# LemonATsu/UNet-PhaseGen

Measured on AMD Instinct MI355X. Metric: spectrogram-frames/sec (train fwd+bwd), higher is better.
Workload: dtype f32; 1 GPU; train.py full step (fwd + cos/sin/mag loss + bwd + Adam), UNetModel(1024, 2048), per-GPU batch 64 x 1024 bins x 256 frames (BASELINE configs[2]); global_batch=64, frames=256, channels=1024, parallelism=dp1, grad_allreduce_payload=fp32, adam=fused into the wgrad epilogues

## Files before the change

### include/phasegen.h

```cpp
#ifndef PHASEGEN_H
#define PHASEGEN_H
#include <stdint.h>

#ifdef __cplusplus
extern "C" {
#endif

#define PG_VERSION 400

enum { PG_OK = 0, PG_ERR_NULL = -1, PG_ERR_SHAPE = -2, PG_ERR_ALIGN = -3, PG_ERR_UNSUPPORTED = -4,
       PG_ERR_WORKSPACE = -5 };

enum { PG_ACT_NONE = 0, PG_ACT_LEAKY02 = 1 , PG_ACT_RELU = 2  };

struct pg_adam_args;
typedef struct pg_conv_args {
    int32_t B, Cin, Cout, Lin, Lout, k, stride, pad;
    const float* x;  int64_t x_bs;
    int32_t x_act;
    int32_t precision;
    const float* w;
    float* y;        int64_t y_bs;
    const float* dy; int64_t dy_bs;
    float* dx;       int64_t dx_bs;
    const float* dx_add; int64_t dx_add_bs;
    const float* dx_ref; int64_t dx_ref_bs;
    int32_t dx_mask;
    int32_t schedule;
    float* dw;
    int32_t y_act; int32_t y2_act;
    float* y2;       int64_t y2_bs;
    void* workspace; int64_t workspace_bytes;
    const struct pg_adam_args* adam;
} pg_conv_args;
int64_t pg_workspace_bytes_conv(void);
enum { PG_PREC_FP32 = 0, PG_PREC_BF16 = 1, PG_PREC_BF16X3 = 2 };
enum { PG_SCHED_AUTO = 0, PG_SCHED_TILE_PER_WG = 1, PG_SCHED_FORCE_STREAMK = 2, PG_SCHED_NO_RAW = 4, PG_SCHED_NO_TALL = 8,
       PG_SCHED_CONTENDED = 16, PG_SCHED_NO_PS = 128, PG_SCHED_NO_RAW3 = 0x2000, PG_SCHED_ALL_RAW3 = 0x4000, PG_SCHED_NO_COLSPLIT = 0x20000, PG_SCHED_COLSPLIT = 0x40000 };
#define PG_SCHED_OVERSUB(f) (((f) & 15) << 8)

int pg_conv1d_fwd(const pg_conv_args* a, void* stream);
int pg_conv1d_dgrad(const pg_conv_args* a, void* stream);
int pg_conv1d_wgrad(const pg_conv_args* a, void* stream);
int pg_convt1d_fwd(const pg_conv_args* a, void* stream);
int pg_convt1d_dgrad(const pg_conv_args* a, void* stream);
int pg_convt1d_wgrad(const pg_conv_args* a, void* stream);
enum { PG_OP_CONV1D_FWD = 0, PG_OP_CONV1D_DGRAD = 1, PG_OP_CONV1D_WGRAD = 2,
       PG_OP_CONVT1D_FWD = 3, PG_OP_CONVT1D_DGRAD = 4, PG_OP_CONVT1D_WGRAD = 5 };
int pg_conv_describe(const pg_conv_args* a, int32_t op, char* buf, int32_t buflen);

// ... 104 lines not shown
```

### unet-phasegen_amd/csrc/conv_common.h

```cpp
#pragma once
#include <hip/hip_runtime.h>
#include <stdint.h>
#include "phasegen.h"
#include "pg_common.h"

namespace pgconv {

struct IgemmParams {
    const float* x; long x_bs;
    const float* w;
    const float* pt; long pt_bs;
    float* y; long y_bs;
    const float* add; long add_bs;
    const float* ref; long ref_bs;
    unsigned x_bytes, w_bytes, pt_bytes;
    int B, Q, M, Lx, Ly, k, s, p;
    int act_x, act_p, mask_mode;
    int U, u_off;
    int LP; float inv_LP;
    int a_vec;
    int tilesM, tilesN;
    int g_ps;
    int tn_stride;
    float* y2; long y2_bs; float y_slope, y2_slope;
    float* ws;
    int nslab;
    int whole;
    int sr;
    int n_lo;
    int x_pitch;
    unsigned short* yh; long yh_bs; int yh_pitch; float yh_slope;
    unsigned short* yh2; long yh2_bs; int yh2_pitch; float yh2_slope;
    float* ad_p; float* ad_m; float* ad_v; PgAdamScalars ad;
};

}
using pgconv::IgemmParams;

namespace {


constexpr int WMB = 4;
constexpr int BM = 64 * WMB, BN = 128, BK = 16, NT = 256;
constexpr int TILE_A = BM * BK, TILE_B = BN * BK;
constexpr int STAGE = TILE_A + TILE_B;
constexpr int AE = BM / 16;

typedef float f32x16 __attribute__((ext_vector_type(16)));
// ... 387 lines not shown
#define PG_STAMP_FLUSH
#define PG_STAMP_DECL
#endif

__device__ __forceinline__ void divmod24(int n, int d, float inv, int& q, int& r) {
    q = (int)((float)n * inv);
    r = n - q * d;
    if (r < 0) { r += d; --q; }
    if (r >= d) { r -= d; ++q; }
}

constexpr int RBM = 128, RBN = 256;
constexpr int RS2 = 768, RS1 = 384;
constexpr int raw_gap(int tj) { return tj >= 8 ? 16 : tj; }
constexpr int RTILE_A = RBM * BK;

enum Kind { KIND_F, KIND_T, KIND_G };

}

namespace pgconv {
hipError_t launch_im2col(int kind, const IgemmParams& p, int grid, hipStream_t st, int prec);
hipError_t launch_raw_ft(int kind, const IgemmParams& p, int grid, hipStream_t st, int prec);
hipError_t launch_raw_ft_tall(int kind, const IgemmParams& p, int grid, hipStream_t st, int prec);
hipError_t launch_raw_g(const IgemmParams& p, int grid, hipStream_t st, int prec);
hipError_t launch_h3(int kind, const IgemmParams& p, int grid, hipStream_t st);
hipError_t launch_h3_fixup(int kind, const IgemmParams& p, int grid, unsigned split_tiles, bool wide, hipStream_t st);
bool raw3_covers(int kind, const IgemmParams& p);
hipError_t launch_raw3(int kind, const IgemmParams& p, int grid, hipStream_t st);
hipError_t launch_raw3_fixup(int kind, const IgemmParams& p, int grid, unsigned blocks, hipStream_t st);
// ... 3 lines not shown
```

### unet-phasegen_amd/csrc/conv_igemm.hip

```cpp
#include <hip/hip_runtime.h>
#include <cstring>
#include <cmath>
#include "conv_common.h"

namespace {

template <int KIND, int MB, int NB, int WN = 2, bool WIDE = false>
__global__ __launch_bounds__(NT) void conv_fixup_kernel(const IgemmParams p, int G) {
    __shared__ float red[WIDE ? 3 * 16 * 64 : 1];
    const int unit = WIDE ? blockIdx.x >> 2 : blockIdx.x, q = WIDE ? threadIdx.x >> 6 : 0;
    const int tid = WIDE ? (blockIdx.x & 3) * 64 + (threadIdx.x & 63) : threadIdx.x;
    const int lane = tid & 63, wv = tid >> 6;
    const int wm = WN == 2 ? wv >> 1 : (WN == 4 ? 0 : wv), wn = WN == 2 ? wv & 1 : (WN == 4 ? wv : 0);
    static_assert(MB * NB * 16 == ACC_REGS, "8 blocks per wave tile: the host launches 8 workgroups per tile");
    const int tile = p.whole + unit / (MB * NB), blk = unit % (MB * NB), bi = blk / NB, bj = blk - bi * NB;
    const Split sp = make_split(p.tilesM * p.tilesN, p.nslab, G, p.whole);
    const int first = tile * p.nslab, last = first + p.nslab - 1;
    const int g0 = split_owner(sp, first), g1 = split_owner(sp, last);
    if (g0 == g1 && split_lo(sp, g0) <= first && split_lo(sp, g0 + 1) > last) return;
    if (KIND != 2 && p.n_lo + (tile % p.tilesN) * p.tn_stride + (WN == 2 ? wn * (NB - 1) * 32 : (WN == 4 ? wn * (NB * 32) : 0)) + bj * 32 >= p.B * (KIND == 0 ? p.Ly : p.U)) return;
    AccT<1, 1> acc;
#pragma unroll
    for (int r = 0; r < 16; ++r) acc.c[0][0][r] = 0.f;
#pragma unroll 2
// ... 31 lines not shown

struct Knobs {
    int prec;
    int force_mode;
    int no_raw;
    int no_tall;
    int oversub;
    int contended;
    int no_ps;
    int no_raw3;
    int all_raw3;
    int sr;
    int force_colsplit;
    int no_colsplit;
    char* desc; int desc_len;
};
int decode_knobs(const pg_conv_args* a, Knobs& k) {
    if (a->precision < 0 || a->precision > 2) return pg_fail(PG_ERR_UNSUPPORTED, "conv: precision must be PG_PREC_FP32, PG_PREC_BF16 or PG_PREC_BF16X3");
    const int sc = a->schedule;
    if (sc < 0 || (sc & ~0x7ffff) || ((sc >> 17) & 3) == 3 || (sc & 3) == 3 || ((sc >> 8) & 15) > 8) return pg_fail(PG_ERR_SHAPE, "conv: bad schedule bits");
    k.prec = a->precision;
    k.force_mode = sc & 3; k.no_raw = (sc >> 2) & 1; k.no_tall = (sc >> 3) & 1;
    k.oversub = (sc >> 8) & 15; if (!k.oversub) k.oversub = 4;
    k.contended = (sc >> 4) & 1;
    if ((sc >> 5) & 3) return pg_fail(PG_ERR_UNSUPPORTED, "conv: schedule bits 5-6 (tile families removed in 0.4)");
    k.no_ps = (sc >> 7) & 1;
    k.no_raw3 = (sc >> 13) & 1;
    k.all_raw3 = (sc >> 14) & 1;
    k.sr = ((sc >> 15) & 3) ? 1 << (((sc >> 15) & 3) - 1) : 0;
    k.no_colsplit = (sc >> 17) & 1;
    k.force_colsplit = (sc >> 18) & 1;
    if (k.no_raw3 && k.all_raw3) return pg_fail(PG_ERR_SHAPE, "conv: schedule bits 13 and 14 exclude each other");
    k.desc = nullptr; k.desc_len = 0;
    return PG_OK;
}

int cu_count() { return pg_cu_count(); }
bool fixup_wide(int grid, long split_tiles) { return split_tiles > 0 && grid >= 8 * split_tiles; }

int pick_grid(long tiles, int nslab, IgemmParams& p, long ws_bytes, int mode, int oversub, int contended, int wg_per_cu = WG_PER_CU,
              long ws_per_wg = WS_PER_WG) {
    const long total = tiles * (long)nslab;
    const long slots = (long)cu_count() * wg_per_cu;
    p.whole = 0;
    if (mode == 0 && !contended && tiles % slots == 0) {
        if (tiles <= slots * oversub) return (int)tiles;
        for (long mult = oversub; mult >= 1; --mult)
            if (tiles % (slots * mult) == 0) return (int)(slots * mult);
// ... 25 lines not shown
    const bool k5 = p.k == 5 && p.s == 2;
    if (kind == KIND_F) {
        if (!((p.k == 32 && p.s == 2) || (p.k == 8 && p.s == 1) || (p.k == 8 && p.s == 2) || (p.k == 4 && p.s == 2) || (k5 && p.Q % 2 == 0))) return false;
        kwp = virtual_k(p.k, p.s); sc = p.s; lcol = p.Ly;
    } else if (kind == KIND_T) {
        if (!((p.k == 32 && p.s == 2) || (p.k == 8 && p.s == 1) || (p.k == 8 && p.s == 2) || (p.k == 4 && p.s == 2) || k5)) return false;
        kwp = virtual_k(p.k, p.s) / p.s; sc = 1; lcol = p.U;
    } else {
        return p.LP >= 16 && ((p.k == 32 && p.s == 2) || (p.k == 8 && p.s == 1) || (p.k == 8 && p.s == 2) || (p.k == 4 && p.s == 2) || k5);
    }
    const int tj = kwp < 16 ? kwp : 16;
    const int nseg_max = (lcol - 1 + tn - 1) / lcol + 1;
    return sc * (tn - 1) + tj + raw_gap(tj) * (nseg_max - 1) + (kind == KIND_T ? tj : 0) <= (sc == 1 ? RS1 : RS2);
}

int launch(Kind kind, IgemmParams& p, const Knobs& kn, long rows, long cols, long Ktot, long ws_bytes, hipStream_t st, bool may_split = true) {
    const long Ktot_in = Ktot;
    bool raw = raw_supported(kind, p, kn);
    const long cols_wide = (cols + RBN - 1) / RBN * RBN, cols_tall = (cols + RBN / 2 - 1) / (RBN / 2) * (RBN / 2);
    const bool tall = kind != KIND_G && kn.no_raw == 0 && kn.no_tall == 0 && (cols_tall * 100 <= cols_wide * 97 || !raw) &&
                      raw_supported(kind, p, kn, RBN / 2);
    if (tall) raw = true;
    const bool r3_over_tall = tall && raw_supported(kind, p, kn) && (kn.all_raw3 || cols_wide * 100 <= cols_tall * 108);
    const bool r3_ok = raw && raw_supported(kind, p, kn) && kind != KIND_G && kn.prec == 0 && !kn.no_raw3 && pgconv::raw3_covers(kind, p) &&
                       (rows + 255) / 256 * 256 * 100 <= (rows + RBM - 1) / RBM * RBM * 103;
    const bool r3 = r3_ok && (!tall || r3_over_tall);
    const int bm = (tall || r3) ? 2 * RBM : (raw ? RBM : BM);
    int bn = (tall && !r3) ? RBN / 2 : (raw ? RBN : BN);
    const bool k5 = raw && p.k == 5 && p.s == 2;
    if (k5 && kind == KIND_G) bn = (RBN / 5) * 5;
    p.g_ps = 0;
    if (raw && kind == KIND_G && p.k != 32) {
// ... 4 lines not shown
    if (may_split && r3_ok && kn.force_mode != 1 && !kn.no_colsplit && !kn.no_tall) {
        const long full = cols / RBN * RBN, rem = cols - full;
        if (full > 0 && rem > 0 && rem <= RBN / 2 && raw_supported(kind, p, kn, RBN / 2)) {
            const double rows_p = (double)((rows + 255) / 256 * 256), rem32 = (double)((rem + 31) / 32 * 32), Kd = (double)Ktot;
            const double t_col = 2.0 * rows_p * 256.0 * Kd / 140e6;
            const double t_tail = fmax(4.0 * (double)rows * Kd / 3e6, 2.0 * rows_p * rem32 * Kd / 100e6) + 25.0;
            IgemmParams pa = p;
            const long tiles_a = (rows + 255) / 256 * (full / RBN), nslab_a = (Ktot + BK - 1) / BK;
            const long grid_a = pick_grid(tiles_a, (int)nslab_a, pa, ws_bytes, kn.force_mode, kn.oversub, kn.contended, 1, 2 * WS_PER_WG);
            const bool aligned = pa.whole == 0 && (grid_a % tiles_a == 0 || tiles_a % grid_a == 0);
            if ((t_col > 1.3 * t_tail && aligned) || kn.force_colsplit) {
                Knobs kb = kn;
                kb.no_raw3 = 1; kb.all_raw3 = 0;
                char tail[160] = "";
                if (kn.desc) { kb.desc = tail; kb.desc_len = (int)sizeof tail; }
                int rc = launch(kind, p, kn, rows, full, Ktot_in, ws_bytes, st, false);
                if (rc != PG_OK) return rc;
                IgemmParams pb = p;
                pb.n_lo = (int)full;
                rc = launch(kind, pb, kb, rows, rem, Ktot_in, ws_bytes, st, false);
                if (rc == PG_OK && kn.desc) {
                    char* bar = strchr(tail, '|');
                    if (bar) { *bar = ','; bar = strchr(bar, '|'); if (bar) *bar = 0; }
                    const size_t n = strlen(kn.desc);
                    if (n + 7 < (size_t)kn.desc_len) snprintf(kn.desc + n, (size_t)kn.desc_len - n, "|tail=%s", tail);
                }
                return rc;
            }
        }
    }
    if (p.n_lo && !(tall && !r3)) return pg_fail(PG_ERR_UNSUPPORTED, "conv: internal -- a column tail off the tall tile");
    p.tn_stride = bn;
    p.sr = r3 ? (kn.sr ? kn.sr : (p.k == 8 ? 2 : 1)) : 0;
    p.tilesM = (int)((rows + bm - 1) / bm);
    p.tilesN = (int)((cols + bn - 1) / bn);
    p.nslab = (int)((Ktot + BK - 1) / BK);
    const long tiles = (long)p.tilesM * p.tilesN;
    if (tiles <= 0 || tiles > 0x0fffffffL || p.nslab <= 0 || cols + bn >= 0x7fffffffL) return pg_fail(PG_ERR_SHAPE, "conv: empty or oversize grid");
    const int grid = r3 ? pick_grid(tiles, p.nslab, p, ws_bytes, kn.force_mode, kn.oversub, kn.contended, 1, 2 * WS_PER_WG)
                        : pick_grid(tiles, p.nslab, p, ws_bytes, kn.force_mode, kn.oversub, kn.contended);
    const bool split = grid != tiles && !(tiles % grid == 0);
    if (kn.desc) {
        char name[96];
        if (raw && kind == KIND_G) snprintf(name, sizeof name, "conv_g_%s_kernel<%d, %d, %d>", p.g_ps ? "ps" : "raw", p.k, p.s, kn.prec);
        else if (r3) snprintf(name, sizeof name, "conv_raw3_kernel<%d, %d, %s, %s>", p.k, p.s, kind == KIND_T ? "true" : "false", p.act_x == PG_ACT_NONE ? "false" : "true");
        else if (raw) snprintf(name, sizeof name, "conv_raw_kernel<%d, %d, %s, %d, %d>", p.k, p.s, kind == KIND_T ? "true" : "false", kn.prec, tall ? 1 : 2);
        else snprintf(name, sizeof name, "conv_%c_kernel<0, 0, %d>", kind == KIND_F ? 'f' : (kind == KIND_T ? 't' : 'g'), kn.prec);
        snprintf(kn.desc, (size_t)kn.desc_len, "%s|grid=%d|tiles=%ld|slabs=%d|split=%d|whole=%d|fixup=%s", name, grid, tiles, p.nslab, (int)split, p.whole,
                 !split ? "none" : (!r3 && fixup_wide(grid, tiles - p.whole) ? "wide" : "plain"));
        return PG_OK;
    }
    hipError_t e;
    if (r3) e = pgconv::launch_raw3(kind, p, grid, st);
    else if (raw && kind == KIND_G) e = pgconv::launch_raw_g(p, grid, st, kn.prec);
    else if (tall) e = pgconv::launch_raw_ft_tall(kind, p, grid, st, kn.prec);
    else if (raw) e = pgconv::launch_raw_ft(kind, p, grid, st, kn.prec);
    else e = pgconv::launch_im2col(kind, p, grid, st, kn.prec);
    if (e == hipSuccess && split && r3) e = pgconv::launch_raw3_fixup(kind, p, grid, (unsigned)((tiles - p.whole) * 16), st);
    else if (e == hipSuccess && split) {
        const bool wide = fixup_wide(grid, tiles - p.whole);
        const dim3 fg((unsigned)((tiles - p.whole) * (wide ? 32 : 8)));
#define PG_FIXUP(...) { if (wide) hipLaunchKernelGGL((conv_fixup_kernel<__VA_ARGS__, true>), fg, dim3(NT), 0, st, p, grid); \
                        else hipLaunchKernelGGL((conv_fixup_kernel<__VA_ARGS__, false>), fg, dim3(NT), 0, st, p, grid); }
        if (tall) {
            if (kind == KIND_F) PG_FIXUP(0, 2, 4, 1)
// ... 118 lines not shown
}

static int set_fused_adam(IgemmParams& p, const pg_conv_args* a) {
    const pg_adam_args* ad = a->adam;
    if (!ad) return PG_OK;
    if (!ad->p || !ad->m || !ad->v) return pg_fail(PG_ERR_NULL, "wgrad: fused adam needs p, m and v");
    if (ad->step < 1) return pg_fail(PG_ERR_SHAPE, "wgrad: fused adam: step is 1-based");
    if (ad->n != (int64_t)a->Cin * a->Cout * a->k) return pg_fail(PG_ERR_SHAPE, "wgrad: fused adam: n must equal Cin * Cout * k (p / m / v shaped like dw)");
    if (((uintptr_t)ad->p | (uintptr_t)ad->m | (uintptr_t)ad->v) & 3) return pg_fail(PG_ERR_ALIGN, "wgrad: fused adam: misaligned pointer");
    if ((const float*)ad->p == a->dw || ad->m == a->dw || ad->v == a->dw) return pg_fail(PG_ERR_SHAPE, "wgrad: fused adam: p / m / v alias dw");
    p.ad_p = ad->p; p.ad_m = ad->m; p.ad_v = ad->v;
    p.ad = pg_adam_scalars(ad);
    return PG_OK;
}

static int run_conv1d_wgrad(const pg_conv_args* a, void* stream, char* desc, int desc_len) {
    if (int e = check_geom(a, false)) return e;
    Knobs kn; if (int e = decode_knobs(a, kn)) return e;
    kn.desc = desc; kn.desc_len = desc_len;
    if (!a->dy || !a->x || !a->dw) return pg_fail(PG_ERR_NULL, "conv1d_wgrad: dy, x, dw required");
    IgemmParams p = {};
    p.pt = a->dy; p.pt_bs = a->dy_bs; p.LP = a->Lout; p.act_p = PG_ACT_NONE;
    p.x = a->x; p.x_bs = a->x_bs; p.act_x = a->x_act; p.y = a->dw;
    p.B = a->B; p.Q = a->Cin; p.M = a->Cout; p.Lx = a->Lin; p.k = a->k; p.s = a->stride; p.p = a->pad;
    if (int e = set_extents(p, p.Q, p.Lx, p.M, p.LP)) return e;
    if (int e = set_fused_adam(p, a)) return e;
    p.ws = (float*)a->workspace;
    return launch(KIND_G, p, kn, p.M, (long)p.Q * p.k, (long)p.B * p.LP, a->workspace_bytes, (hipStream_t)stream);
}

static int run_convt1d_wgrad(const pg_conv_args* a, void* stream, char* desc, int desc_len) {
    if (int e = check_geom(a, true)) return e;
    Knobs kn; if (int e = decode_knobs(a, kn)) return e;
    kn.desc = desc; kn.desc_len = desc_len;
    if (!a->dy || !a->x || !a->dw) return pg_fail(PG_ERR_NULL, "convt1d_wgrad: dy, x, dw required");
    IgemmParams p = {};
    p.pt = a->x; p.pt_bs = a->x_bs; p.LP = a->Lin; p.act_p = a->x_act;
    p.x = a->dy; p.x_bs = a->dy_bs; p.act_x = PG_ACT_NONE; p.y = a->dw;
    p.B = a->B; p.Q = a->Cout; p.M = a->Cin; p.Lx = a->Lout; p.k = a->k; p.s = a->stride; p.p = a->pad;
    if (int e = set_extents(p, p.Q, p.Lx, p.M, p.LP)) return e;
    if (int e = set_fused_adam(p, a)) return e;
    p.ws = (float*)a->workspace;
    return launch(KIND_G, p, kn, p.M, (long)p.Q * p.k, (long)p.B * p.LP, a->workspace_bytes, (hipStream_t)stream);
}

extern "C" int pg_conv1d_fwd(const pg_conv_args* a, void* stream) { return run_conv1d_fwd(a, stream, nullptr, 0); }
extern "C" int pg_conv1d_dgrad(const pg_conv_args* a, void* stream) { return run_conv1d_dgrad(a, stream, nullptr, 0); }
extern "C" int pg_conv1d_wgrad(const pg_conv_args* a, void* stream) { return run_conv1d_wgrad(a, stream, nullptr, 0); }
extern "C" int pg_convt1d_fwd(const pg_conv_args* a, void* stream) { return run_convt1d_fwd(a, stream, nullptr, 0); }
extern "C" int pg_convt1d_dgrad(const pg_conv_args* a, void* stream) { return run_convt1d_dgrad(a, stream, nullptr, 0); }
// ... 48 lines not shown
        p.u_off = p.p / p.s;
        p.U = (p.Ly - 1 + p.p) / p.s - p.u_off + 1;
        if (p.U <= 0) return pg_fail(PG_ERR_SHAPE, "conv_fwd_h: empty output");
    }
    if (!pgconv::h_supported(kind, p)) return pg_fail(PG_ERR_UNSUPPORTED, "conv_fwd_h: geometry not covered by the bf16-resident kernels (use the fp32-tensor entry points)");
    if (query) return PG_OK;
    const long rows = tr ? (long)p.M * p.s : p.M, cols = (long)p.B * (tr ? p.U : p.Ly), Ktot = (long)p.Q * kwp;
    const int tm = 2 * RBM, tn = RBN;
    p.tilesM = (int)((rows + tm - 1) / tm);
    p.tilesN = (int)((cols + tn - 1) / tn);
    p.tn_stride = tn;
    p.nslab = (int)(Ktot / 32);
    p.ws = (float*)a->workspace;
    const long tiles = (long)p.tilesM * p.tilesN;
    if (tiles <= 0 || tiles > 0x0fffffffL || p.nslab <= 0) return pg_fail(PG_ERR_SHAPE, "conv_fwd_h: empty or oversize grid");
    const int grid = pick_grid(tiles, p.nslab, p, a->workspace_bytes, kn.force_mode, kn.oversub, kn.contended, 1, 2 * WS_PER_WG);
    const bool split = grid != tiles && !(tiles % grid == 0);
    if (desc) {
        snprintf(desc, (size_t)desc_len, "conv_h3_kernel<%d, %d, %s>|grid=%d|tiles=%ld|slabs=%d|split=%d|whole=%d|fixup=%s",
                 (tr && p.k == 5) ? 8 : p.k, p.s, tr ? "true" : "false", grid, tiles, p.nslab, (int)split, p.whole,
                 !split ? "none" : (fixup_wide(grid, tiles - p.whole) ? "wide" : "plain"));
        return PG_OK;
    }
    hipStream_t st = (hipStream_t)stream;
    hipError_t e = pgconv::launch_h3(kind, p, grid, st);
    if (e == hipSuccess && split) e = pgconv::launch_h3_fixup(kind, p, grid, (unsigned)(tiles - p.whole), fixup_wide(grid, tiles - p.whole), st);
    if (e != hipSuccess) return pg_fail((int)e, hipGetErrorString(e));
    return PG_OK;
}

extern "C" int pg_conv_fwd_h(const pg_convh_args* a, void* stream) { return conv_fwd_h_impl(a, stream, false); }
extern "C" int pg_conv_fwd_h_supported(const pg_convh_args* a) { return conv_fwd_h_impl(a, nullptr, true) == PG_OK ? 1 : 0; }
extern "C" int pg_conv_fwd_h_describe(const pg_convh_args* a, char* buf, int32_t buflen) {
    if (!buf || buflen < 128) return pg_fail(PG_ERR_NULL, "conv_fwd_h_describe: buf of >= 128 bytes required");
    buf[0] = 0;
    return conv_fwd_h_impl(a, nullptr, false, buf, buflen);
}

extern "C" int64_t pg_workspace_bytes_conv(void) { return (int64_t)MAX_STREAMK_WG * WS_PER_WG; }
```

### unet-phasegen_amd/csrc/conv_raw_wgrad.hip

```cpp
#include "conv_common.h"

namespace {

template <int KW, int S> struct GRaw {
    static constexpr int WL = 15 * S + KW;
    static constexpr int WLP = (KW == 32) ? 64 : (KW == 8 ? (S == 1 ? 24 : 40) : 36);
    static constexpr int NQT = RBN / KW;
    static constexpr int TNV = NQT * KW;
    static constexpr int SUB = NQT * WLP;
    static constexpr int SUBS = (SUB + 63) / 64 * 64;
    static constexpr int NE = (SUB + NT - 1) / NT;
    static constexpr int STG = RTILE_A + 2 * SUBS;
    static_assert(WL <= WLP, "window does not fit its slot");
};

template <int KW, int S, int BF>
__global__ __launch_bounds__(NT, 2) void conv_g_raw_kernel(const IgemmParams p) {
    using C = GRaw<KW, S>;
    __shared__ __attribute__((aligned(16))) float lds[2 * C::STG];
    const int tid = threadIdx.x, lane = tid & 63;
    const int wv = __builtin_amdgcn_readfirstlane(tid >> 6), wm = wv >> 1, wn = wv & 1;
    const int kt = dma_kt(lane, wv);
    const rsrc_t rp = make_rsrc(p.pt, p.pt_bytes), rx = make_rsrc(p.x, p.x_bytes);
    const float slopeA = act_slope(p.act_p), slopeB = act_slope(p.act_x);
    const int pbs4 = (int)p.pt_bs * 4, xbs4 = (int)p.x_bs * 4;
    const int g = logical_wg(blockIdx.x, gridDim.x, p.whole);
    const Split sp = make_split(p.tilesM * p.tilesN, p.nslab, gridDim.x, p.whole);
    int pos = split_lo(sp, g);
    const int pos_end = split_lo(sp, g + 1);
    int slot = 0;
    while (pos < pos_end) {
        const int tile = pos / p.nslab, sb = pos - tile * p.nslab;
// ... 180 lines not shown
#endif
            PG_STAMP(3)
        }
        PG_STAMP_FLUSH
#undef GRAW_ISSUE
#undef GRAW_CHOFF
#undef GRAW_VV
        if (sb == 0 && se == p.nslab) epilogue_g<S, 2, 4>(p, acc, m0, n0, lane, wm, wn, n0 + C::TNV);
        else store_partial(p.ws, g, slot, acc, tid);
        pos += se - sb;
        slot = 1;
    }
}

template <int KW, int S, int BF>
__global__ __launch_bounds__(NT, 2) void conv_g_ps_kernel(const IgemmParams p) {
    using C = GRaw<KW, S>;
    constexpr int STG = RTILE_A + (C::SUB + 255) / 256 * 256;
    constexpr int NE16 = (C::SUB / 4 + NT - 1) / NT;
    static_assert(C::WLP % 4 == 0 && C::WLP <= 64, "16-byte window pieces; channel 0 inside the first 64 floats");
    __shared__ __attribute__((aligned(16))) float lds[2 * STG];
    const int tid = threadIdx.x, lane = tid & 63;
    const int wv = __builtin_amdgcn_readfirstlane(tid >> 6), wm = wv >> 1, wn = wv & 1;
    const rsrc_t rp = make_rsrc(p.pt, p.pt_bytes), rx = make_rsrc(p.x, p.x_bytes);
    const float slopeA = act_slope(p.act_p), slopeB = act_slope(p.act_x);
    const int pbs4 = (int)p.pt_bs * 4, xbs4 = (int)p.x_bs * 4;
    const int cps = (p.LP + 15) >> 4;
    const int g = logical_wg(blockIdx.x, gridDim.x, p.whole);
    const Split sp = make_split(p.tilesM * p.tilesN, p.nslab, gridDim.x, p.whole);
    int pos = split_lo(sp, g);
    const int pos_end = split_lo(sp, g + 1);
// ... 119 lines not shown
            }
            __builtin_amdgcn_sched_barrier(0);
            if (++mc == cps) { mc = 0; ++mb; }
            __syncthreads();
        }
#undef GPS_ISSUE
        (void)mb;
        if (sb == 0 && se == p.nslab) epilogue_g<S, 2, 4>(p, acc, m0, n0, lane, wm, wn, n0 + C::TNV);
        else store_partial(p.ws, g, slot, acc, tid);
        pos += se - sb;
        slot = 1;
    }
}

template <int KW, int S>
hipError_t launch_g_raw(const IgemmParams& p, int grid, hipStream_t st, int prec) {
    if (p.g_ps) {
        if (prec == 1) hipLaunchKernelGGL((conv_g_ps_kernel<KW, S, 1>), dim3(grid), dim3(NT), 0, st, p);
        else if (prec == 2) hipLaunchKernelGGL((conv_g_ps_kernel<KW, S, 2>), dim3(grid), dim3(NT), 0, st, p);
        else hipLaunchKernelGGL((conv_g_ps_kernel<KW, S, 0>), dim3(grid), dim3(NT), 0, st, p);
        return hipGetLastError();
    }
    if (prec == 1) hipLaunchKernelGGL((conv_g_raw_kernel<KW, S, 1>), dim3(grid), dim3(NT), 0, st, p);
    else if (prec == 2) hipLaunchKernelGGL((conv_g_raw_kernel<KW, S, 2>), dim3(grid), dim3(NT), 0, st, p);
    else hipLaunchKernelGGL((conv_g_raw_kernel<KW, S, 0>), dim3(grid), dim3(NT), 0, st, p);
    return hipGetLastError();
}

}

hipError_t pgconv::launch_raw_g(const IgemmParams& p, int grid, hipStream_t st, int prec) {
// ... 7 lines not shown
```

### unet-phasegen_amd/phasegen/_lib.py

```python
import ctypes as C
import os

_HERE = os.path.dirname(os.path.abspath(__file__))
LIB_PATH = os.path.join(_HERE, "libphasegen.so")
ABI_VERSION = 400

ACT_NONE, ACT_LEAKY, ACT_RELU = 0, 1, 2
PREC_FP32, PREC_BF16, PREC_BF16X3 = 0, 1, 2
OK, ERR_NULL, ERR_SHAPE, ERR_ALIGN, ERR_UNSUPPORTED, ERR_WORKSPACE = 0, -1, -2, -3, -4, -5
OP_CONV1D_FWD, OP_CONV1D_DGRAD, OP_CONV1D_WGRAD, OP_CONVT1D_FWD, OP_CONVT1D_DGRAD, OP_CONVT1D_WGRAD = range(6)
SCHED_AUTO, SCHED_TILE_PER_WG, SCHED_FORCE_STREAMK, SCHED_NO_RAW, SCHED_NO_TALL, SCHED_CONTENDED = 0, 1, 2, 4, 8, 16
SCHED_NO_PS = 128
SCHED_NO_RAW3 = 0x2000
SCHED_ALL_RAW3 = 0x4000
SCHED_NO_COLSPLIT = 0x20000
SCHED_COLSPLIT = 0x40000

c_float_p = C.c_void_p


class ConvArgs(C.Structure):
    _fields_ = [("B", C.c_int32), ("Cin", C.c_int32), ("Cout", C.c_int32), ("Lin", C.c_int32), ("Lout", C.c_int32),
                ("k", C.c_int32), ("stride", C.c_int32), ("pad", C.c_int32),
                ("x", C.c_void_p), ("x_bs", C.c_int64), ("x_act", C.c_int32), ("precision", C.c_int32),
# ... 90 lines not shown
    "pg_conv1d_dgrad": (C.c_int, [C.POINTER(ConvArgs), C.c_void_p]),
    "pg_conv1d_wgrad": (C.c_int, [C.POINTER(ConvArgs), C.c_void_p]),
    "pg_convt1d_fwd": (C.c_int, [C.POINTER(ConvArgs), C.c_void_p]),
    "pg_convt1d_dgrad": (C.c_int, [C.POINTER(ConvArgs), C.c_void_p]),
    "pg_convt1d_wgrad": (C.c_int, [C.POINTER(ConvArgs), C.c_void_p]),
    "pg_conv_describe": (C.c_int, [C.POINTER(ConvArgs), C.c_int32, C.c_char_p, C.c_int32]),
    "pg_conv_fwd_h": (C.c_int, [C.POINTER(ConvhArgs), C.c_void_p]),
    "pg_conv_fwd_h_supported": (C.c_int, [C.POINTER(ConvhArgs)]),
    "pg_workspace_bytes_moments": (C.c_int64, []),
    "pg_moments": (C.c_int, [C.POINTER(MomentsArgs), C.c_void_p]),
    "pg_standardize": (C.c_int, [C.c_void_p, C.c_int64, C.c_void_p, C.c_void_p]),
    "pg_shadow_elems": (C.c_int64, [C.c_int32, C.c_int32, C.c_int32, C.c_int32, C.c_int32]),
    "pg_shadow_weights": (C.c_int, [C.c_void_p, C.c_void_p, C.c_int32, C.c_int32, C.c_int32, C.c_int32, C.c_int32, C.c_void_p]),
    "pg_cast_rows_bf16": (C.c_int, [C.POINTER(CastArgs), C.c_void_p]),
    "pg_workspace_bytes_conv": (C.c_int64, []),
    "pg_bn_fwd": (C.c_int, [C.POINTER(BnArgs), C.c_void_p]),
    "pg_bn_bwd": (C.c_int, [C.POINTER(BnArgs), C.c_void_p]),
    "pg_workspace_bytes_loss": (C.c_int64, [C.POINTER(LossArgs)]),
    "pg_loss_fwd_bwd": (C.c_int, [C.POINTER(LossArgs), C.c_void_p]),
    "pg_adam_step": (C.c_int, [C.POINTER(AdamArgs), C.c_void_p]),
    "pg_stft": (C.c_int, [C.POINTER(StftArgs), C.c_void_p]),
    "pg_stft_frame_index": (C.c_int, [C.c_int32, C.c_int32, C.c_int32, C.c_int32, C.c_void_p, C.c_void_p]),
    "pg_polar": (C.c_int, [C.POINTER(PolarArgs), C.c_void_p]),
    "pg_workspace_bytes_istft": (C.c_int64, [C.POINTER(IstftArgs)]),
    "pg_istft": (C.c_int, [C.POINTER(IstftArgs), C.c_void_p]),
    "pg_gl_project": (C.c_int, [C.POINTER(GlArgs), C.c_void_p]),
    "pg_ola_nt": (C.c_int, [C.POINTER(OlaArgs), C.c_void_p]),
    "pg_fill": (C.c_int, [C.c_void_p, C.c_int64, C.c_float, C.c_void_p]),
    "pg_conv_fwd_h_describe": (C.c_int, [C.POINTER(ConvhArgs), C.c_char_p, C.c_int32]),
    "pg_version": (C.c_int, []),
# ... 31 lines not shown
```

### unet-phasegen_amd/phasegen/ops.py

```python
import contextlib
import ctypes as C
import threading

import torch

from . import _lib
from ._lib import ACT_LEAKY, ACT_NONE, ACT_RELU, SCHED_CONTENDED, SCHED_TILE_PER_WG


def _stream():
    return C.c_void_p(torch.cuda.current_stream().cuda_stream)


def _on_current_device(t, name):
    if t.device.index != torch.cuda.current_device():
        raise ValueError(f"{name}: tensor is on {t.device} but the current device is cuda:{torch.cuda.current_device()} "
                         "(wrap the call in torch.cuda.device(...))")


class KernelTimer:

    def __init__(self):
        self.records = {}
        self.plans = {}
# ... 254 lines not shown
def conv_wgrad(x, dy, dw, stride, pad, x_act=ACT_NONE, transposed=False, precision=None, schedule=None, adam=None):
    Cin, Cout, k = _geom(transposed, dw)
    B, _, Lin = x.shape
    a = _conv_args(transposed, B, Cin, Cout, Lin, k, stride, pad, x.device, precision, schedule)
    if tuple(x.shape) != (B, Cin, Lin) or tuple(dy.shape) != (B, Cout, a.Lout):
        raise ValueError(f"conv_wgrad: shapes x{tuple(x.shape)} dy{tuple(dy.shape)} dw{tuple(dw.shape)} inconsistent")
    a.x, a.x_bs = _act3(x, "x")
    a.dy, a.dy_bs = _act3(dy, "dy")
    a.dw = _dense(dw, "dw")
    a.x_act = x_act
    if adam is not None:
        if adam.n != dw.numel():
            raise ValueError("conv_wgrad: fused adam tensors must have dw's shape")
        a.adam = C.addressof(adam)
    lib = _lib.load()
    _note_plan(a, _lib.OP_CONVT1D_WGRAD if transposed else _lib.OP_CONV1D_WGRAD)
    fn = lib.pg_convt1d_wgrad if transposed else lib.pg_conv1d_wgrad
    _lib.check(fn(C.byref(a), _stream()), "wgrad")
    return dw


H_HEAD = 32
H_TAIL = 40


def h_pitch(L):
    return (L + H_TAIL + 7) // 8 * 8


def h_alloc(B, Cc, L, device):
    pitch = h_pitch(L)
# ... 292 lines not shown
```

Before: 97350 frames/s.

## Pre-pack fp32 wgrad operands into padded workspace buffers for raw kernels

For fp32 weight-gradient convolutions on the raw path, this adds pack kernels that copy x (with padding and activation applied) and dy into contiguous padded row layouts in an extended workspace. New fp32 raw and ps kernel bodies then read these packed buffers through buffer DMA without per-element bounds or activation handling, and the workspace query API grows to size the extra buffers. This trades extra pack passes and memory traffic for simpler, aligned 16-byte loads in the main GEMM loop.

```diff
diff --git a/include/phasegen.h b/include/phasegen.h
--- a/include/phasegen.h
+++ b/include/phasegen.h
@@ -34,6 +34,7 @@
     const struct pg_adam_args* adam;
 } pg_conv_args;
 int64_t pg_workspace_bytes_conv(void);
+int64_t pg_workspace_bytes_wgrad(const pg_conv_args* a, int32_t op);
 enum { PG_PREC_FP32 = 0, PG_PREC_BF16 = 1, PG_PREC_BF16X3 = 2 };
 enum { PG_SCHED_AUTO = 0, PG_SCHED_TILE_PER_WG = 1, PG_SCHED_FORCE_STREAMK = 2, PG_SCHED_NO_RAW = 4, PG_SCHED_NO_TALL = 8,
        PG_SCHED_CONTENDED = 16, PG_SCHED_NO_PS = 128, PG_SCHED_NO_RAW3 = 0x2000, PG_SCHED_ALL_RAW3 = 0x4000, PG_SCHED_NO_COLSPLIT = 0x20000, PG_SCHED_COLSPLIT = 0x40000 };
diff --git a/unet-phasegen_amd/csrc/conv_common.h b/unet-phasegen_amd/csrc/conv_common.h
--- a/unet-phasegen_amd/csrc/conv_common.h
+++ b/unet-phasegen_amd/csrc/conv_common.h
@@ -32,6 +32,8 @@
     unsigned short* yh; long yh_bs; int yh_pitch; float yh_slope;
     unsigned short* yh2; long yh2_bs; int yh2_pitch; float yh2_slope;
     float* ad_p; float* ad_m; float* ad_v; PgAdamScalars ad;
+    const float* qk; unsigned qk_bytes; int qk_bs, Lq;
+    const float* pk; unsigned pk_bytes; int Kp;
 };
 
 }
@@ -449,6 +451,7 @@
 constexpr int RS2 = 768, RS1 = 384;
 constexpr int raw_gap(int tj) { return tj >= 8 ? 16 : tj; }
 constexpr int RTILE_A = RBM * BK;
+constexpr int g_wlp(int kw, int s) { return kw == 32 ? 64 : (kw == 8 ? (s == 1 ? 24 : 40) : 36); }
 
 enum Kind { KIND_F, KIND_T, KIND_G };
 
diff --git a/unet-phasegen_amd/csrc/conv_igemm.hip b/unet-phasegen_amd/csrc/conv_igemm.hip
--- a/unet-phasegen_amd/csrc/conv_igemm.hip
+++ b/unet-phasegen_amd/csrc/conv_igemm.hip
@@ -1,6 +1,7 @@
 #include <hip/hip_runtime.h>
 #include <cstring>
 #include <cmath>
+#include <algorithm>
 #include "conv_common.h"
 
 namespace {
@@ -69,6 +70,7 @@
     int force_colsplit;
     int no_colsplit;
     char* desc; int desc_len;
+    long* pack_need;
 };
 int decode_knobs(const pg_conv_args* a, Knobs& k) {
     if (a->precision < 0 || a->precision > 2) return pg_fail(PG_ERR_UNSUPPORTED, "conv: precision must be PG_PREC_FP32, PG_PREC_BF16 or PG_PREC_BF16X3");
@@ -86,7 +88,7 @@
     k.no_colsplit = (sc >> 17) & 1;
     k.force_colsplit = (sc >> 18) & 1;
     if (k.no_raw3 && k.all_raw3) return pg_fail(PG_ERR_SHAPE, "conv: schedule bits 13 and 14 exclude each other");
-    k.desc = nullptr; k.desc_len = 0;
+    k.desc = nullptr; k.desc_len = 0; k.pack_need = nullptr;
     return PG_OK;
 }
 
@@ -142,8 +144,26 @@
     return sc * (tn - 1) + tj + raw_gap(tj) * (nseg_max - 1) + (kind == KIND_T ? tj : 0) <= (sc == 1 ? RS1 : RS2);
 }
 
+constexpr long WS_STREAMK = (long)MAX_STREAMK_WG * WS_PER_WG;
+
+long g_pack_layout(IgemmParams& p) {
+    const int cps = (p.LP + 15) / 16;
+    const long gimax = p.g_ps ? 16L * (cps - 1) : (long)p.LP - 1;
+    long lq = (long)p.s * gimax + g_wlp(p.k, p.s);
+    if (lq < (long)p.p + p.Lx) lq = (long)p.p + p.Lx;
+    lq = (lq + 3) / 4 * 4;
+    const long kp = p.g_ps ? 16L * cps : 16L * p.nslab;
+    const long qbytes = (long)p.B * p.Q * lq * 4, pbytes = (p.g_ps ? (long)p.B : 1L) * p.M * kp * 4;
+    if (qbytes >= 0x7ffffff0L || pbytes >= 0x7ffffff0L) return -1;
+    p.Lq = (int)lq; p.qk_bs = (int)((long)p.Q * lq); p.qk_bytes = (unsigned)qbytes;
+    p.Kp = (int)kp; p.pk_bytes = (unsigned)pbytes;
+    return (qbytes + 255) / 256 * 256 + pbytes;
+}
+
 int launch(Kind kind, IgemmParams& p, const Knobs& kn, long rows, long cols, long Ktot, long ws_bytes, hipStream_t st, bool may_split = true) {
     const long Ktot_in = Ktot;
+    const long ws_all = ws_bytes;
+    if (ws_bytes > WS_STREAMK) ws_bytes = WS_STREAMK;
     bool raw = raw_supported(kind, p, kn);
     const long cols_wide = (cols + RBN - 1) / RBN * RBN, cols_tall = (cols + RBN / 2 - 1) / (RBN / 2) * (RBN / 2);
     const bool tall = kind != KIND_G && kn.no_raw == 0 && kn.no_tall == 0 && (cols_tall * 100 <= cols_wide * 97 || !raw) &&
@@ -178,11 +198,11 @@
                 kb.no_raw3 = 1; kb.all_raw3 = 0;
                 char tail[160] = "";
                 if (kn.desc) { kb.desc = tail; kb.desc_len = (int)sizeof tail; }
-                int rc = launch(kind, p, kn, rows, full, Ktot_in, ws_bytes, st, false);
+                int rc = launch(kind, p, kn, rows, full, Ktot_in, ws_all, st, false);
                 if (rc != PG_OK) return rc;
                 IgemmParams pb = p;
                 pb.n_lo = (int)full;
-                rc = launch(kind, pb, kb, rows, rem, Ktot_in, ws_bytes, st, false);
+                rc = launch(kind, pb, kb, rows, rem, Ktot_in, ws_all, st, false);
                 if (rc == PG_OK && kn.desc) {
                     char* bar = strchr(tail, '|');
                     if (bar) { *bar = ','; bar = strchr(bar, '|'); if (bar) *bar = 0; }
@@ -201,6 +221,10 @@
     p.nslab = (int)((Ktot + BK - 1) / BK);
     const long tiles = (long)p.tilesM * p.tilesN;
     if (tiles <= 0 || tiles > 0x0fffffffL || p.nslab <= 0 || cols + bn >= 0x7fffffffL) return pg_fail(PG_ERR_SHAPE, "conv: empty or oversize grid");
+    const bool packed = raw && kind == KIND_G && kn.prec == 0;
+    const long pack = packed ? g_pack_layout(p) : 0;
+    if (pack < 0) return pg_fail(PG_ERR_SHAPE, "wgrad: packed operand exceeds 2 GiB (31-bit buffer offsets)");
+    if (kn.pack_need) { *kn.pack_need = pack; return PG_OK; }
     const int grid = r3 ? pick_grid(tiles, p.nslab, p, ws_bytes, kn.force_mode, kn.oversub, kn.contended, 1, 2 * WS_PER_WG)
                         : pick_grid(tiles, p.nslab, p, ws_bytes, kn.force_mode, kn.oversub, kn.contended);
     const bool split = grid != tiles && !(tiles % grid == 0);
@@ -213,6 +237,12 @@
         snprintf(kn.desc, (size_t)kn.desc_len, "%s|grid=%d|tiles=%ld|slabs=%d|split=%d|whole=%d|fixup=%s", name, grid, tiles, p.nslab, (int)split, p.whole,
                  !split ? "none" : (!r3 && fixup_wide(grid, tiles - p.whole) ? "wide" : "plain"));
         return PG_OK;
+    }
+    if (packed) {
+        if (!p.ws || ws_all < WS_STREAMK + pack)
+            return pg_fail(PG_ERR_WORKSPACE, "wgrad: the fp32 kernels need pg_workspace_bytes_wgrad() bytes of workspace (packed operands)");
+        p.qk = reinterpret_cast<const float*>(reinterpret_cast<char*>(p.ws) + WS_STREAMK);
+        p.pk = reinterpret_cast<const float*>(reinterpret_cast<const char*>(p.qk) + ((long)p.qk_bytes + 255) / 256 * 256);
     }
     hipError_t e;
     if (r3) e = pgconv::launch_raw3(kind, p, grid, st);
@@ -361,11 +391,11 @@
     return PG_OK;
 }
 
-static int run_conv1d_wgrad(const pg_conv_args* a, void* stream, char* desc, int desc_len) {
+static int run_conv1d_wgrad(const pg_conv_args* a, void* stream, char* desc, int desc_len, long* pack_need = nullptr) {
     if (int e = check_geom(a, false)) return e;
     Knobs kn; if (int e = decode_knobs(a, kn)) return e;
-    kn.desc = desc; kn.desc_len = desc_len;
-    if (!a->dy || !a->x || !a->dw) return pg_fail(PG_ERR_NULL, "conv1d_wgrad: dy, x, dw required");
+    kn.desc = desc; kn.desc_len = desc_len; kn.pack_need = pack_need;
+    if (!pack_need && (!a->dy || !a->x || !a->dw)) return pg_fail(PG_ERR_NULL, "conv1d_wgrad: dy, x, dw required");
     IgemmParams p = {};
     p.pt = a->dy; p.pt_bs = a->dy_bs; p.LP = a->Lout; p.act_p = PG_ACT_NONE;
     p.x = a->x; p.x_bs = a->x_bs; p.act_x = a->x_act; p.y = a->dw;
@@ -376,11 +406,11 @@
     return launch(KIND_G, p, kn, p.M, (long)p.Q * p.k, (long)p.B * p.LP, a->workspace_bytes, (hipStream_t)stream);
 }
 
-static int run_convt1d_wgrad(const pg_conv_args* a, void* stream, char* desc, int desc_len) {
+static int run_convt1d_wgrad(const pg_conv_args* a, void* stream, char* desc, int desc_len, long* pack_need = nullptr) {
     if (int e = check_geom(a, true)) return e;
     Knobs kn; if (int e = decode_knobs(a, kn)) return e;
-    kn.desc = desc; kn.desc_len = desc_len;
-    if (!a->dy || !a->x || !a->dw) return pg_fail(PG_ERR_NULL, "convt1d_wgrad: dy, x, dw required");
+    kn.desc = desc; kn.desc_len = desc_len; kn.pack_need = pack_need;
+    if (!pack_need && (!a->dy || !a->x || !a->dw)) return pg_fail(PG_ERR_NULL, "convt1d_wgrad: dy, x, dw required");
     IgemmParams p = {};
     p.pt = a->x; p.pt_bs = a->x_bs; p.LP = a->Lin; p.act_p = a->x_act;
     p.x = a->dy; p.x_bs = a->dy_bs; p.act_x = PG_ACT_NONE; p.y = a->dw;
@@ -459,7 +489,7 @@
     p.ws = (float*)a->workspace;
     const long tiles = (long)p.tilesM * p.tilesN;
     if (tiles <= 0 || tiles > 0x0fffffffL || p.nslab <= 0) return pg_fail(PG_ERR_SHAPE, "conv_fwd_h: empty or oversize grid");
-    const int grid = pick_grid(tiles, p.nslab, p, a->workspace_bytes, kn.force_mode, kn.oversub, kn.contended, 1, 2 * WS_PER_WG);
+    const int grid = pick_grid(tiles, p.nslab, p, std::min((long)a->workspace_bytes, WS_STREAMK), kn.force_mode, kn.oversub, kn.contended, 1, 2 * WS_PER_WG);
     const bool split = grid != tiles && !(tiles % grid == 0);
     if (desc) {
         snprintf(desc, (size_t)desc_len, "conv_h3_kernel<%d, %d, %s>|grid=%d|tiles=%ld|slabs=%d|split=%d|whole=%d|fixup=%s",
@@ -482,4 +512,12 @@
     return conv_fwd_h_impl(a, nullptr, false, buf, buflen);
 }
 
-extern "C" int64_t pg_workspace_bytes_conv(void) { return (int64_t)MAX_STREAMK_WG * WS_PER_WG; }
+extern "C" int64_t pg_workspace_bytes_conv(void) { return (int64_t)WS_STREAMK; }
+extern "C" int64_t pg_workspace_bytes_wgrad(const pg_conv_args* a, int32_t op) {
+    long need = 0;
+    int e;
+    if (op == PG_OP_CONV1D_WGRAD) e = run_conv1d_wgrad(a, nullptr, nullptr, 0, &need);
+    else if (op == PG_OP_CONVT1D_WGRAD) e = run_convt1d_wgrad(a, nullptr, nullptr, 0, &need);
+    else return pg_fail(PG_ERR_UNSUPPORTED, "workspace_bytes_wgrad: op must be PG_OP_CONV1D_WGRAD or PG_OP_CONVT1D_WGRAD");
+    return e != PG_OK ? (int64_t)e : (int64_t)(WS_STREAMK + need);
+}
diff --git a/unet-phasegen_amd/csrc/conv_raw_wgrad.hip b/unet-phasegen_amd/csrc/conv_raw_wgrad.hip
--- a/unet-phasegen_amd/csrc/conv_raw_wgrad.hip
+++ b/unet-phasegen_amd/csrc/conv_raw_wgrad.hip
@@ -4,18 +4,19 @@
 
 template <int KW, int S> struct GRaw {
     static constexpr int WL = 15 * S + KW;
-    static constexpr int WLP = (KW == 32) ? 64 : (KW == 8 ? (S == 1 ? 24 : 40) : 36);
+    static constexpr int WLP = g_wlp(KW, S);
     static constexpr int NQT = RBN / KW;
     static constexpr int TNV = NQT * KW;
     static constexpr int SUB = NQT * WLP;
     static constexpr int SUBS = (SUB + 63) / 64 * 64;
     static constexpr int NE = (SUB + NT - 1) / NT;
     static constexpr int STG = RTILE_A + 2 * SUBS;
+    static constexpr int SUBP = (SUB + 255) / 256 * 256;
     static_assert(WL <= WLP, "window does not fit its slot");
 };
 
 template <int KW, int S, int BF>
-__global__ __launch_bounds__(NT, 2) void conv_g_raw_kernel(const IgemmParams p) {
+__device__ __forceinline__ void g_raw_bf(const IgemmParams& p) {
     using C = GRaw<KW, S>;
     __shared__ __attribute__((aligned(16))) float lds[2 * C::STG];
     const int tid = threadIdx.x, lane = tid & 63;
@@ -226,7 +227,7 @@
 }
 
 template <int KW, int S, int BF>
-__global__ __launch_bounds__(NT, 2) void conv_g_ps_kernel(const IgemmParams p) {
+__device__ __forceinline__ void g_ps_bf(const IgemmParams& p) {
     using C = GRaw<KW, S>;
     constexpr int STG = RTILE_A + (C::SUB + 255) / 256 * 256;
     constexpr int NE16 = (C::SUB / 4 + NT - 1) / NT;
@@ -376,7 +377,292 @@
 }
 
 template <int KW, int S>
+__device__ __forceinline__ void g_raw_f32(const IgemmParams& p) {
+    using C = GRaw<KW, S>;
+    constexpr int NP = 2 * C::SUBP / 4;
+    constexpr int NE2 = (NP + NT - 1) / NT;
+    constexpr int STG = RTILE_A + 2 * C::SUBP;
+    static_assert(C::WLP % 4 == 0 && 2 * STG * 4 <= 64 * 1024, "16-byte window pieces; LDS budget");
+    __shared__ __attribute__((aligned(16))) float lds[2 * STG];
+    const int tid = threadIdx.x, lane = tid & 63;
+    const int wv = __builtin_amdgcn_readfirstlane(tid >> 6), wm = wv >> 1, wn = wv & 1;
+    const rsrc_t rp = make_rsrc(p.pk, p.pk_bytes), rx = make_rsrc(p.qk, p.qk_bytes);
+    const int qbs4 = p.qk_bs * 4, klast4 = (p.nslab - 1) * BK * 4;
+    const int g = logical_wg(blockIdx.x, gridDim.x, p.whole);
+    const Split sp = make_split(p.tilesM * p.tilesN, p.nslab, gridDim.x, p.whole);
+    int pos = split_lo(sp, g);
+    const int pos_end = split_lo(sp, g + 1);
+    int slot = 0;
+    while (pos < pos_end) {
+        const int tile = pos / p.nslab, sb = pos - tile * p.nslab;
+        const int se = min(p.nslab, sb + (pos_end - pos));
+        const int m0 = (tile / p.tilesN) * RBM, n0 = (tile % p.tilesN) * C::TNV;
+        const int qbase = (tile % p.tilesN) * C::NQT;
+        int pv[2], woff[NE2];
+#pragma unroll
+        for (int e = 0; e < 2; ++e) {
+            const int m = m0 + dma16_row(lane, wv, e);
+            pv[e] = m < p.M ? (m * p.Kp + dma16_kc(lane)) * 4 : FAR;
+        }
+#pragma unroll
+        for (int e = 0; e < NE2; ++e) {
+            const int pc = tid + NT * e, sub = pc >= C::SUBP / 4 ? 1 : 0, f = 4 * pc - sub * C::SUBP, ql = f / C::WLP, v0 = f - ql * C::WLP;
+            woff[e] = (f < C::SUB && qbase + ql < p.Q) ? ((qbase + ql) * p.Lq + v0) * 4 : FAR;
+        }
+        int bbase[4];
+#pragma unroll
+        for (int jb = 0; jb < 4; ++jb) {
+            const int c = wn * 128 + jb * 32 + (lane & 31), qc = c / KW;
+            bbase[jb] = qc * C::WLP + (c - qc * KW) + S * 8 * (lane >> 5);
+        }
+        AccR acc;
+#pragma unroll
+        for (int i = 0; i < 2; ++i)
+#pragma unroll
+            for (int j = 0; j < 4; ++j)
+#pragma unroll
+                for (int r = 0; r < 16; ++r) acc.c[i][j][r] = 0.f;
+
+        int gb, gi;
+        { const int k0 = sb * BK; gb = k0 / p.LP; gi = k0 - gb * p.LP; }
+        int kc_cur, kc_next;
+#define GRF_ISSUE(STAGE_PTR, K0)                                                                          \
+    {   const int sa = min((K0) * 4, klast4);                                                             \
+        _Pragma("unroll") for (int e = 0; e < 2; ++e) dma16s(rp, (STAGE_PTR) + wv * 256 + e * 1024, pv[e], sa); \
+        const int kc = p.LP - gi;                                                                         \
+        const int sw0 = min(gb, p.B - 1) * qbs4 + S * gi * 4;                                             \
+        const int sw1 = (kc < 16 && gb + 1 < p.B) ? (gb + 1) * qbs4 : sw0;                                \
+        _Pragma("unroll") for (int e = 0; e < NE2; ++e) {                                                 \
+            const int pc0 = e * NT + wv * 64;                                 \
+            if ((e + 1) * NT <= NP || pc0 < NP)                                                           \
+                dma16s(rx, (STAGE_PTR) + RTILE_A + 4 * pc0, woff[e], pc0 >= C::SUBP / 4 ? sw1 : sw0);     \
+        }                                                                                                 \
+        kc_next = kc < 16 ? kc : 16;                                                                      \
+        gi += BK; if (gi >= p.LP) { gi -= p.LP; ++gb; }                                                   \
+    }
+        PG_STAMP_DECL
+        GRF_ISSUE(lds, sb * BK)
+        kc_cur = kc_next;
+        __syncthreads();
+        for (int sl = sb; sl < se; ++sl) {
+            const int cur = (sl - sb) & 1;
+            PG_STAMP(0)
+#if defined(PG_G_ABL) && PG_G_ABL == 1
+            kc_next = 16;
+#else
+            GRF_ISSUE(lds + (cur ^ 1) * STG, (sl + 1) * BK)
+#endif
+            __builtin_amdgcn_sched_barrier(0);
+            PG_STAMP(1)
+            {
+                const float* As = lds + cur * STG;
+                const float* Bw = As + RTILE_A;
+                const int r = lane & 31, h = lane >> 5, sw = (r >> 2) & 3;
+                const float* ap = As + (wm * 64 + r) * BK;
+                f32x4 a[2][2];
+                float b[4][8];
+                if (kc_cur >= 16) {
+#pragma unroll
+                    for (int i = 0; i < 2; ++i) a[i][0] = *reinterpret_cast<const f32x4*>(ap + i * 32 * BK + (((2 * h) ^ sw) << 2));
+#pragma unroll
+                    for (int ip = 0; ip < 4; ++ip) {
+                        if (ip == 2) {
+#pragma unroll
+                            for (int i = 0; i < 2; ++i) a[i][1] = *reinterpret_cast<const f32x4*>(ap + i * 32 * BK + (((2 * h + 1) ^ sw) << 2));
+                        }
+#pragma unroll
+                        for (int jb = 0; jb < 4; ++jb) { b[jb][2 * ip] = Bw[bbase[jb] + S * 2 * ip]; b[jb][2 * ip + 1] = Bw[bbase[jb] + S * (2 * ip + 1)]; }
+                    }
+                } else {
+#pragma unroll
+                    for (int c = 0; c < 2; ++c)
+#pragma unroll
+                        for (int i = 0; i < 2; ++i) a[i][c] = *reinterpret_cast<const f32x4*>(ap + i * 32 * BK + (((2 * h + c) ^ sw) << 2));
+                    typedef const volatile __attribute__((address_space(3))) float* lds_vptr;
+                    const lds_vptr Bv = (lds_vptr)Bw;
+                    const int shift = C::SUBP - S * kc_cur;
+#pragma unroll
+                    for (int i = 0; i < 8; ++i) {
+                        const int d = (8 * h + i >= kc_cur) ? shift : 0;
+#pragma unroll
+                        for (int jb = 0; jb < 4; ++jb) b[jb][i] = Bv[bbase[jb] + S * i + d];
+                    }
+                }
+#pragma unroll
+                for (int kk = 0; kk < 8; ++kk)
+#pragma unroll
+                    for (int i = 0; i < 2; ++i)
+#pragma unroll
+                        for (int j = 0; j < 4; ++j)
+                            acc.c[i][j] = __builtin_amdgcn_mfma_f32_32x32x2f32(a[i][kk >> 2][kk & 3], b[j][kk], acc.c[i][j], 0, 0, 0);
+            }
+            __builtin_amdgcn_sched_barrier(0);
+            PG_STAMP(2)
+            kc_cur = kc_next;
+            __syncthreads();
+            PG_STAMP(3)
+        }
+        PG_STAMP_FLUSH
+#undef GRF_ISSUE
+        if (sb == 0 && se == p.nslab) epilogue_g<S, 2, 4>(p, acc, m0, n0, lane, wm, wn, n0 + C::TNV);
+        else store_partial(p.ws, g, slot, acc, tid);
+        pos += se - sb;
+        slot = 1;
+    }
+}
+
+template <int KW, int S>
+__device__ __forceinline__ void g_ps_f32(const IgemmParams& p) {
+    using C = GRaw<KW, S>;
+    constexpr int STG = RTILE_A + (C::SUB + 255) / 256 * 256;
+    constexpr int NE16 = (C::SUB / 4 + NT - 1) / NT;
+    static_assert(C::WLP % 4 == 0, "16-byte window pieces");
+    __shared__ __attribute__((aligned(16))) float lds[2 * STG];
+    const int tid = threadIdx.x, lane = tid & 63;
+    const int wv = __builtin_amdgcn_readfirstlane(tid >> 6), wm = wv >> 1, wn = wv & 1;
+    const rsrc_t rp = make_rsrc(p.pk, p.pk_bytes), rx = make_rsrc(p.qk, p.qk_bytes);
+    const int pbs4 = p.M * p.Kp * 4, qbs4 = p.qk_bs * 4;
+    const int cps = p.Kp >> 4;
+    const int g = logical_wg(blockIdx.x, gridDim.x, p.whole);
+    const Split sp = make_split(p.tilesM * p.tilesN, p.nslab, gridDim.x, p.whole);
+    int pos = split_lo(sp, g);
+    const int pos_end = split_lo(sp, g + 1);
+    int slot = 0;
+    while (pos < pos_end) {
+        const int tile = pos / p.nslab, sb = pos - tile * p.nslab;
+        const int se = min(p.nslab, sb + (pos_end - pos));
+        const int m0 = (tile / p.tilesN) * RBM, n0 = (tile % p.tilesN) * C::TNV;
+        const int qbase = (tile % p.tilesN) * C::NQT;
+        int pv[2], woff[NE16];
+#pragma unroll
+        for (int e = 0; e < 2; ++e) {
+            const int m = m0 + dma16_row(lane, wv, e);
+            pv[e] = m < p.M ? (m * p.Kp + dma16_kc(lane)) * 4 : FAR;
+        }
+#pragma unroll
+        for (int e = 0; e < NE16; ++e) {
+            const int f = 4 * (tid + NT * e), ql = f / C::WLP, v0 = f - ql * C::WLP;
+            woff[e] = (f < C::SUB && qbase + ql < p.Q) ? ((qbase + ql) * p.Lq + v0) * 4 : FAR;
+        }
+        int bbase[4];
+#pragma unroll
+        for (int jb = 0; jb < 4; ++jb) {
+            const int c = wn * 128 + jb * 32 + (lane & 31), qc = c / KW;
+            bbase[jb] = qc * C::WLP + (c - qc * KW) + S * 8 * (lane >> 5);
+        }
+        AccR acc;
+#pragma unroll
+        for (int i = 0; i < 2; ++i)
+#pragma unroll
+            for (int j = 0; j < 4; ++j)
+#pragma unroll
+                for (int r = 0; r < 16; ++r) acc.c[i][j][r] = 0.f;
+
+        int gb = sb / cps, gc = sb - gb * cps;
+#define GPF_ISSUE(STAGE_PTR)                                                                              \
+    {   const int gbc = min(gb, p.B - 1), gi = gc << 4;                                                   \
+        _Pragma("unroll") for (int e = 0; e < 2; ++e) dma16s(rp, (STAGE_PTR) + wv * 256 + e * 1024, pv[e], gbc * pbs4 + gi * 4); \
+        const int sw_ = gbc * qbs4 + S * gi * 4;                                                          \
+        _Pragma("unroll") for (int e = 0; e < NE16; ++e)                                                  \
+            if (4 * (e * NT + wv * 64) < C::SUB) dma16s(rx, (STAGE_PTR) + RTILE_A + 4 * (e * NT + wv * 64), woff[e], sw_); \
+        if (++gc == cps) { gc = 0; ++gb; }                                                                \
+    }
+        GPF_ISSUE(lds)
+        __syncthreads();
+        for (int sl = sb; sl < se; ++sl) {
+            const int cur = (sl - sb) & 1;
+            GPF_ISSUE(lds + (cur ^ 1) * STG)
+            __builtin_amdgcn_sched_barrier(0);
+            {
+                const float* As = lds + cur * STG;
+                const float* Bw = As + RTILE_A;
+                const int r = lane & 31, h = lane >> 5, sw = (r >> 2) & 3;
+                const float* ap = As + (wm * 64 + r) * BK;
+                f32x4 a[2][2];
+                float b[4][8];
+#pragma unroll
+                for (int i = 0; i < 2; ++i) a[i][0] = *reinterpret_cast<const f32x4*>(ap + i * 32 * BK + (((2 * h) ^ sw) << 2));
+#pragma unroll
+                for (int ip = 0; ip < 4; ++ip) {
+                    if (ip == 2) {
+#pragma unroll
+                        for (int i = 0; i < 2; ++i) a[i][1] = *reinterpret_cast<const f32x4*>(ap + i * 32 * BK + (((2 * h + 1) ^ sw) << 2));
+                    }
+#pragma unroll
+                    for (int jb = 0; jb < 4; ++jb) { b[jb][2 * ip] = Bw[bbase[jb] + S * 2 * ip]; b[jb][2 * ip + 1] = Bw[bbase[jb] + S * (2 * ip + 1)]; }
+                }
+#pragma unroll
+                for (int kk = 0; kk < 8; ++kk)
+#pragma unroll
+                    for (int i = 0; i < 2; ++i)
+#pragma unroll
+                        for (int j = 0; j < 4; ++j)
+                            acc.c[i][j] = __builtin_amdgcn_mfma_f32_32x32x2f32(a[i][kk >> 2][kk & 3], b[j][kk], acc.c[i][j], 0, 0, 0);
+            }
+            __builtin_amdgcn_sched_barrier(0);
+            __syncthreads();
+        }
+#undef GPF_ISSUE
+        if (sb == 0 && se == p.nslab) epilogue_g<S, 2, 4>(p, acc, m0, n0, lane, wm, wn, n0 + C::TNV);
+        else store_partial(p.ws, g, slot, acc, tid);
+        pos += se - sb;
+        slot = 1;
+    }
+}
+
+template <int KW, int S, int BF>
+__global__ __launch_bounds__(NT, 2) void conv_g_raw_kernel(const IgemmParams p) {
+    if constexpr (BF == 0) g_raw_f32<KW, S>(p);
+    else g_raw_bf<KW, S, BF>(p);
+}
+template <int KW, int S, int BF>
+__global__ __launch_bounds__(NT, 2) void conv_g_ps_kernel(const IgemmParams p) {
+    if constexpr (BF == 0) g_ps_f32<KW, S>(p);
+    else g_ps_bf<KW, S, BF>(p);
+}
+
+__global__ __launch_bounds__(256) void pack_rows_kernel(const float* __restrict__ src, long bs, int C, int L, int F, int W, unsigned n,
+                                                       float slope, float* __restrict__ dst) {
+    for (unsigned i = blockIdx.x * 256u + threadIdx.x; i < n; i += gridDim.x * 256u) {
+        const unsigned r = i / (unsigned)W, b = r / (unsigned)C, c = r - b * (unsigned)C;
+        const int t = (int)(i - r * (unsigned)W) - F;
+        float v = 0.f;
+        if ((unsigned)t < (unsigned)L) {
+            v = src[(long)b * bs + (long)c * L + t];
+            if (slope != 1.0f) v = act_apply(v, slope);
+        }
+        dst[i] = v;
+    }
+}
+__global__ __launch_bounds__(256) void pack_flat_kernel(const float* __restrict__ src, long bs, int B, int LP, int Kp, unsigned n,
+                                                       float slope, float* __restrict__ dst) {
+    for (unsigned i = blockIdx.x * 256u + threadIdx.x; i < n; i += gridDim.x * 256u) {
+        const unsigned m = i / (unsigned)Kp, k = i - m * (unsigned)Kp, b = k / (unsigned)LP, t = k - b * (unsigned)LP;
+        float v = 0.f;
+        if ((int)b < B) {
+            v = src[(long)b * bs + (long)m * LP + t];
+            if (slope != 1.0f) v = act_apply(v, slope);
+        }
+        dst[i] = v;
+    }
+}
+unsigned pack_grid(unsigned n) { return (n + 255u) / 256u < 2048u ? (n + 255u) / 256u : 2048u; }
+
+hipError_t pack_g(const IgemmParams& p, hipStream_t st) {
+    float* const qk = const_cast<float*>(p.qk);
+    float* const pk = const_cast<float*>(p.pk);
+    const unsigned nq = (unsigned)(p.qk_bytes / 4), np = (unsigned)(p.pk_bytes / 4);
+    hipLaunchKernelGGL(pack_rows_kernel, dim3(pack_grid(nq)), dim3(256), 0, st, p.x, p.x_bs, p.Q, p.Lx, p.p, p.Lq, nq, act_slope(p.act_x), qk);
+    if (p.g_ps) hipLaunchKernelGGL(pack_rows_kernel, dim3(pack_grid(np)), dim3(256), 0, st, p.pt, p.pt_bs, p.M, p.LP, 0, p.Kp, np, act_slope(p.act_p), pk);
+    else hipLaunchKernelGGL(pack_flat_kernel, dim3(pack_grid(np)), dim3(256), 0, st, p.pt, p.pt_bs, p.B, p.LP, p.Kp, np, act_slope(p.act_p), pk);
+    return hipGetLastError();
+}
+
+template <int KW, int S>
 hipError_t launch_g_raw(const IgemmParams& p, int grid, hipStream_t st, int prec) {
+    if (prec == 0) {
+        if (hipError_t e = pack_g(p, st)) return e;
+    }
     if (p.g_ps) {
         if (prec == 1) hipLaunchKernelGGL((conv_g_ps_kernel<KW, S, 1>), dim3(grid), dim3(NT), 0, st, p);
         else if (prec == 2) hipLaunchKernelGGL((conv_g_ps_kernel<KW, S, 2>), dim3(grid), dim3(NT), 0, st, p);
diff --git a/unet-phasegen_amd/phasegen/_lib.py b/unet-phasegen_amd/phasegen/_lib.py
--- a/unet-phasegen_amd/phasegen/_lib.py
+++ b/unet-phasegen_amd/phasegen/_lib.py
@@ -128,6 +128,7 @@
     "pg_shadow_weights": (C.c_int, [C.c_void_p, C.c_void_p, C.c_int32, C.c_int32, C.c_int32, C.c_int32, C.c_int32, C.c_void_p]),
     "pg_cast_rows_bf16": (C.c_int, [C.POINTER(CastArgs), C.c_void_p]),
     "pg_workspace_bytes_conv": (C.c_int64, []),
+    "pg_workspace_bytes_wgrad": (C.c_int64, [C.POINTER(ConvArgs), C.c_int32]),
     "pg_bn_fwd": (C.c_int, [C.POINTER(BnArgs), C.c_void_p]),
     "pg_bn_bwd": (C.c_int, [C.POINTER(BnArgs), C.c_void_p]),
     "pg_workspace_bytes_loss": (C.c_int64, [C.POINTER(LossArgs)]),
diff --git a/unet-phasegen_amd/phasegen/ops.py b/unet-phasegen_amd/phasegen/ops.py
--- a/unet-phasegen_amd/phasegen/ops.py
+++ b/unet-phasegen_amd/phasegen/ops.py
@@ -292,7 +292,12 @@
             raise ValueError("conv_wgrad: fused adam tensors must have dw's shape")
         a.adam = C.addressof(adam)
     lib = _lib.load()
-    _note_plan(a, _lib.OP_CONVT1D_WGRAD if transposed else _lib.OP_CONV1D_WGRAD)
+    op = _lib.OP_CONVT1D_WGRAD if transposed else _lib.OP_CONV1D_WGRAD
+    need = lib.pg_workspace_bytes_wgrad(C.byref(a), op)
+    if need > a.workspace_bytes:
+        ws = _conv_ws.get(x.device, lib.pg_workspace_bytes_conv, at_least=need)
+        a.workspace, a.workspace_bytes = ws.data_ptr(), ws.numel()
+    _note_plan(a, op)
     fn = lib.pg_convt1d_wgrad if transposed else lib.pg_conv1d_wgrad
     _lib.check(fn(C.byref(a), _stream()), "wgrad")
     return dw
```

Result: faster. 98840 frames/s (median of 6 runs) (+1.5%).
